# aminrezaee/mujoco_reinforcement_learning

Measured on NVIDIA B200. Metric: ppo_update_samples_per_sec, higher is better.
Workload: dtype bf16

## Files before the change

### mujoco_reinforcement_learning_b200/build.py

```python
from __future__ import annotations

import os
import subprocess
import sys
from concurrent.futures import ThreadPoolExecutor

HERE = os.path.dirname(os.path.abspath(__file__))
ROOT = os.path.dirname(HERE)
CSRC = os.path.join(HERE, "csrc")
INCLUDE = os.path.join(ROOT, "include")
BUILD_DIR = os.path.join(HERE, "build")
LIB_PATH = os.path.join(HERE, "libb200ppo.so")

NVCC_FLAGS = [
    "-gencode", "arch=compute_100a,code=sm_100a", "-lineinfo", "-O3", "-std=c++17",
    "-Xcompiler", "-fPIC", "-Xcompiler", "-fvisibility=hidden", f"-I{INCLUDE}", f"-I{CSRC}",
]


def _sources():
    return sorted(os.path.join(CSRC, f) for f in os.listdir(CSRC) if f.endswith(".cu"))


def _newest_input():
    deps = [os.path.join(CSRC, f) for f in os.listdir(CSRC)] + [os.path.join(INCLUDE, "b200ppo.h"), __file__]
    return max(os.path.getmtime(p) for p in deps)


def needs_build() -> bool:
    return not os.path.exists(LIB_PATH) or os.path.getmtime(LIB_PATH) < _newest_input()


def build_library(force: bool = False, verbose: bool = False) -> str:
    if not force and not needs_build():
        return LIB_PATH
    nvcc = os.environ.get("NVCC", "/usr/local/cuda/bin/nvcc")
    os.makedirs(BUILD_DIR, exist_ok=True)

    def compile_one(src):
        obj = os.path.join(BUILD_DIR, os.path.basename(src)[:-3] + ".o")
        cmd = [nvcc, *NVCC_FLAGS, "-c", src, "-o", obj]
        if verbose:
            cmd.insert(1, "-Xptxas=-v")
        res = subprocess.run(cmd, capture_output=True, text=True)
        if res.returncode != 0:
            raise RuntimeError(f"nvcc failed for {src}:\n{res.stdout}\n{res.stderr}")
        if verbose:
            sys.stderr.write(res.stderr)
        return obj

    with ThreadPoolExecutor(max_workers=min(8, os.cpu_count() or 1)) as ex:
        objs = list(ex.map(compile_one, _sources()))
    tmp = LIB_PATH + ".tmp"
    res = subprocess.run([nvcc, "-shared", "-gencode", "arch=compute_100a,code=sm_100a", "-o", tmp, *objs, "-ldl"],
                         capture_output=True, text=True)
    if res.returncode != 0:
        raise RuntimeError(f"link failed:\n{res.stdout}\n{res.stderr}")
    os.replace(tmp, LIB_PATH)
    return LIB_PATH


if __name__ == "__main__":
    path = build_library(force="--force" in sys.argv, verbose="-v" in sys.argv)
    print(path)
```

### mujoco_reinforcement_learning_b200/csrc/adam.cu

```cuda
#include <math.h>

#include "adam.cuh"

namespace b200ppo {

__device__ __forceinline__ void adam_update(float& p, float g, float& m, float& v, const AdamScalars& s) {
  m = __fadd_rn(m, __fmul_rn(s.one_minus_b1, __fsub_rn(g, m)));
  v = __fadd_rn(__fmul_rn(v, s.b2), __fmul_rn(__fmul_rn(s.one_minus_b2, g), g));
  const float denom = __fadd_rn(__fdiv_rn(__fsqrt_rn(v), s.bc2_sqrt), s.eps);
  p = __fadd_rn(p, __fmul_rn(s.neg_step_size, __fdiv_rn(m, denom)));
}

__global__ void __launch_bounds__(256)
adam_kernel(float* __restrict__ params, const float* __restrict__ grads, int n_partials, int64_t partial_stride,
            float* __restrict__ exp_avg, float* __restrict__ exp_avg_sq, int64_t n, int64_t seg_split,
            AdamScalars s0, AdamScalars s1, float* __restrict__ grad_out) {
  const int64_t tid = int64_t(blockIdx.x) * blockDim.x + threadIdx.x;
  const int64_t nthreads = int64_t(gridDim.x) * blockDim.x;
  const int64_t n4 = n >> 2;
  for (int64_t i = tid; i < n4; i += nthreads) {
    float4 g = *reinterpret_cast<const float4*>(grads + 4 * i);
    for (int k = 1; k < n_partials; ++k) {
      const float4 h = *reinterpret_cast<const float4*>(grads + k * partial_stride + 4 * i);
      g.x += h.x; g.y += h.y; g.z += h.z; g.w += h.w;
    }
    float4 p = *reinterpret_cast<float4*>(params + 4 * i);
    float4 m = *reinterpret_cast<float4*>(exp_avg + 4 * i);
    float4 v = *reinterpret_cast<float4*>(exp_avg_sq + 4 * i);
    const int64_t e = 4 * i;
    adam_update(p.x, g.x, m.x, v.x, e + 0 < seg_split ? s0 : s1);
    adam_update(p.y, g.y, m.y, v.y, e + 1 < seg_split ? s0 : s1);
    adam_update(p.z, g.z, m.z, v.z, e + 2 < seg_split ? s0 : s1);
    adam_update(p.w, g.w, m.w, v.w, e + 3 < seg_split ? s0 : s1);
    *reinterpret_cast<float4*>(params + 4 * i) = p;
    *reinterpret_cast<float4*>(exp_avg + 4 * i) = m;
    *reinterpret_cast<float4*>(exp_avg_sq + 4 * i) = v;
    if (grad_out != nullptr) *reinterpret_cast<float4*>(grad_out + 4 * i) = g;
  }
  for (int64_t e = 4 * n4 + tid; e < n; e += nthreads) {
    float g = grads[e];
    for (int k = 1; k < n_partials; ++k) g += grads[k * partial_stride + e];
    float p = params[e], m = exp_avg[e], v = exp_avg_sq[e];
    adam_update(p, g, m, v, e < seg_split ? s0 : s1);
    params[e] = p; exp_avg[e] = m; exp_avg_sq[e] = v;
    if (grad_out != nullptr) grad_out[e] = g;
  }
}

__device__ __forceinline__ void add_partials(float4& g, const float* __restrict__ grads, int k0, int n_partials, int64_t partial_stride, int64_t i) {
  constexpr int NB = 8;
  for (; k0 < n_partials; k0 += NB) {
    float4 h[NB];
#pragma unroll
    for (int j = 0; j < NB; ++j)
      if (k0 + j < n_partials) h[j] = __ldg(reinterpret_cast<const float4*>(grads + int64_t(k0 + j) * partial_stride + 4 * i));
#pragma unroll
    for (int j = 0; j < NB; ++j)
      if (k0 + j < n_partials) { g.x += h[j].x; g.y += h[j].y; g.z += h[j].z; g.w += h[j].w; }
  }
}

struct CastTable {
  int64_t begin[2 * B200PPO_MAX_LAYERS], end[2 * B200PPO_MAX_LAYERS];
  __nv_bfloat16* dst[2 * B200PPO_MAX_LAYERS];
  int in[2 * B200PPO_MAX_LAYERS], pitch[2 * B200PPO_MAX_LAYERS];
  int count;
};

__device__ __forceinline__ void combine_losses(const LossCombine& lc, float* s_lc, float* s_scr) {
  const int tid = threadIdx.x;
  const float s = combine_partials<256>(lc.partials, unsigned(lc.n_cta), 2 + lc.act_dim, tid, s_scr);
  if (tid < 2 + lc.act_dim) s_lc[tid] = tid < 2 ? s : s - lc.ent_coef * lc.rank_share / float(lc.act_dim);
  if (tid == 0 && lc.losses_out != nullptr) {
    float ent = 0.f;
    for (int j = 0; j < lc.act_dim; ++j) ent += 0.5f + 0.91893853320467274178f + logf(expf(lc.logstd[j]));
    ent /= float(lc.act_dim);
    lc.losses_out[0] = -s * lc.inv_global_batch - lc.ent_coef * ent * lc.rank_share;
  }
  if (tid == 1 && lc.losses_out != nullptr) lc.losses_out[1] = s * lc.inv_global_batch;
  __syncthreads();
}

__device__ __forceinline__ bool peer_exchange_barrier(const PeerSrc& ps) {
  const int q = threadIdx.x;
  int timed_out = 0;
  if (q < ps.world && q != ps.rank) {
    if (blockIdx.x == 0) {
      if (ps.local_out != nullptr) {
        const long long t0 = clock64();
        unsigned d;
        do {
          asm volatile("ld.acquire.gpu.global.u32 %0, [%1];" : "=r"(d) : "l"(ps.done_counter) : "memory");
        } while (int(d - ps.done_target) < 0 && clock64() - t0 <= ps.timeout_cycles);
      }
      __threadfence_system();
      asm volatile("st.release.sys.global.u32 [%0], %1;" ::"l"(ps.flags_peer[q] + ps.rank), "r"(ps.seq) : "memory");
    }
    const long long t0 = clock64();
    unsigned v;
    do {
      asm volatile("ld.acquire.sys.global.u32 %0, [%1];" : "=r"(v) : "l"(ps.flags_local + q) : "memory");
      if (clock64() - t0 > ps.timeout_cycles) {
        if (ps.err != nullptr) atomicMax(ps.err, B200PPO_ERRFLAG_PEER_TIMEOUT);
        timed_out = 1;
        break;
      }
    } while (int(v - ps.seq) < 0);
  }
  return __syncthreads_or(timed_out) == 0;
}

__device__ __forceinline__ float4 ld_peer4(const float* p) {
  float4 r;
  asm volatile("ld.volatile.global.v4.f32 {%0,%1,%2,%3}, [%4];" : "=f"(r.x), "=f"(r.y), "=f"(r.z), "=f"(r.w) : "l"(p) : "memory");
  return r;
}

template <bool PEERS>
__global__ void __launch_bounds__(256, 3)
adam_cast_kernel(float* __restrict__ params, const float* __restrict__ grads, int n_partials, int64_t partial_stride,
                 float* __restrict__ exp_avg, float* __restrict__ exp_avg_sq, int64_t n, int64_t seg_split, AdamScalars s0,
                 AdamScalars s1, const __grid_constant__ CastTable ct, const __grid_constant__ LossCombine lc,
                 const __grid_constant__ PeerSrc ps) {
  __shared__ float s_lc[64];
  __shared__ float s_scr[256];
  pdl_wait_then_release();
  const int64_t tid = int64_t(blockIdx.x) * blockDim.x + threadIdx.x;
  const int64_t nthreads = int64_t(gridDim.x) * blockDim.x;
  const int64_t n4 = n >> 2;
  const bool lc_owner = lc.partials != nullptr && int64_t(blockIdx.x) == ((lc.logstd_off >> 2) / blockDim.x) % gridDim.x;
  if (lc_owner) combine_losses(lc, s_lc, s_scr);
  float4 g_local = make_float4(0.f, 0.f, 0.f, 0.f);
  bool fused = false;
  if constexpr (PEERS) {
    fused = ps.local_out != nullptr;
    if (fused) {
      if (tid < n4) {
        g_local = __ldg(reinterpret_cast<const float4*>(grads + 4 * tid));
        add_partials(g_local, grads, 1, n_partials, partial_stride, tid);
        if (lc_owner && 4 * tid + 3 >= lc.logstd_off && 4 * tid < lc.logstd_off + lc.act_dim) {
          const int64_t r = 4 * tid - lc.logstd_off;
          if (r + 0 >= 0 && r + 0 < lc.act_dim) g_local.x = s_lc[2 + r + 0];
          if (r + 1 >= 0 && r + 1 < lc.act_dim) g_local.y = s_lc[2 + r + 1];
          if (r + 2 >= 0 && r + 2 < lc.act_dim) g_local.z = s_lc[2 + r + 2];
          if (r + 3 >= 0 && r + 3 < lc.act_dim) g_local.w = s_lc[2 + r + 3];
        }
        *reinterpret_cast<float4*>(ps.local_out + 4 * tid) = g_local;
      }
      __threadfence();
      __syncthreads();
      if (threadIdx.x == 0) atomicAdd(ps.done_counter, 1u);
    }
    if (!peer_exchange_barrier(ps)) return;
    if (blockIdx.x == 0 && threadIdx.x < 2 && ps.losses_out != nullptr) {
      float l = 0.f;
      for (int r = 0; r < ps.world; ++r) {
        float t;
        asm volatile("ld.volatile.global.f32 %0, [%1];" : "=f"(t) : "l"(ps.src[r] + n + threadIdx.x) : "memory");
        l += t;
      }
      ps.losses_out[threadIdx.x] = l;
    }
  }
  for (int64_t i = tid; i < n4; i += nthreads) {
    const float4 p0 = *reinterpret_cast<float4*>(params + 4 * i);
    const float4 m0 = *reinterpret_cast<float4*>(exp_avg + 4 * i);
    const float4 v0 = *reinterpret_cast<float4*>(exp_avg_sq + 4 * i);
    float4 g;
    if constexpr (PEERS) {
      float4 h[kMaxPeers];
#pragma unroll
      for (int r = 0; r < kMaxPeers; ++r)
        if (r < ps.world) h[r] = (fused && r == ps.rank) ? g_local : ld_peer4(ps.src[r] + 4 * i);
      g = h[0];
#pragma unroll
      for (int r = 1; r < kMaxPeers; ++r)
        if (r < ps.world) { g.x += h[r].x; g.y += h[r].y; g.z += h[r].z; g.w += h[r].w; }
    } else {
      g = *reinterpret_cast<const float4*>(grads + 4 * i);
    }
    if constexpr (!PEERS) add_partials(g, grads, 1, n_partials, partial_stride, i);
    if (!PEERS && lc_owner && 4 * i + 3 >= lc.logstd_off && 4 * i < lc.logstd_off + lc.act_dim) {
      const int64_t r = 4 * i - lc.logstd_off;
      if (r + 0 >= 0 && r + 0 < lc.act_dim) g.x = s_lc[2 + r + 0];
      if (r + 1 >= 0 && r + 1 < lc.act_dim) g.y = s_lc[2 + r + 1];
      if (r + 2 >= 0 && r + 2 < lc.act_dim) g.z = s_lc[2 + r + 2];
      if (r + 3 >= 0 && r + 3 < lc.act_dim) g.w = s_lc[2 + r + 3];
    }
    float4 p = p0, m = m0, v = v0;
    const int64_t e = 4 * i;
    adam_update(p.x, g.x, m.x, v.x, e + 0 < seg_split ? s0 : s1);
    adam_update(p.y, g.y, m.y, v.y, e + 1 < seg_split ? s0 : s1);
    adam_update(p.z, g.z, m.z, v.z, e + 2 < seg_split ? s0 : s1);
    adam_update(p.w, g.w, m.w, v.w, e + 3 < seg_split ? s0 : s1);
    *reinterpret_cast<float4*>(params + 4 * i) = p;
    *reinterpret_cast<float4*>(exp_avg + 4 * i) = m;
    *reinterpret_cast<float4*>(exp_avg_sq + 4 * i) = v;
    int k = -1;
#pragma unroll 1
    for (int c = 0; c < ct.count; ++c)
      if (e >= ct.begin[c] && e < ct.end[c]) k = c;
    if (k >= 0 && (ct.in[k] & 3) == 0 && (ct.pitch[k] & 3) == 0 && e + 3 < ct.end[k]) {
      const uint32_t in = uint32_t(ct.in[k]), rel = uint32_t(e - ct.begin[k]);
      const uint32_t o = rel / in, c2 = rel - o * in;
      const __nv_bfloat162 lo = __floats2bfloat162_rn(p.x, p.y), hi = __floats2bfloat162_rn(p.z, p.w);
      uint2 w;
      w.x = *reinterpret_cast<const uint32_t*>(&lo);
      w.y = *reinterpret_cast<const uint32_t*>(&hi);
      *reinterpret_cast<uint2*>(ct.dst[k] + int64_t(o) * ct.pitch[k] + c2) = w;
    } else if (k >= 0) {
      const float pv[4] = {p.x, p.y, p.z, p.w};
      const int in = ct.in[k];
      const int64_t rel = e - ct.begin[k];
#pragma unroll
      for (int j = 0; j < 4; ++j) {
        if (e + j >= ct.end[k]) break;
        const int o = int((rel + j) / in), c2 = int((rel + j) - int64_t(o) * in);
        ct.dst[k][int64_t(o) * ct.pitch[k] + c2] = __float2bfloat16_rn(pv[j]);
      }
    }
  }
}

__global__ void __launch_bounds__(256)
reduce_partials_kernel(const float* __restrict__ grads, int n_partials, int64_t partial_stride, int64_t n,
                       float* __restrict__ out, const __grid_constant__ LossCombine lc, int vec4) {
  __shared__ float s_lc[64];
  __shared__ float s_scr[256];
  pdl_wait_then_release();
  const int64_t tid = int64_t(blockIdx.x) * blockDim.x + threadIdx.x;
  const int64_t nthreads = int64_t(gridDim.x) * blockDim.x;
  const int64_t n4 = vec4 ? (n >> 2) : 0;
  const bool lc_owner = lc.partials != nullptr && int64_t(blockIdx.x) == (vec4 ? ((lc.logstd_off >> 2) / blockDim.x) % gridDim.x
                                                                               : (lc.logstd_off / blockDim.x) % gridDim.x);
  if (lc_owner) combine_losses(lc, s_lc, s_scr);
  for (int64_t i = tid; i < n4; i += nthreads) {
    float4 g = *reinterpret_cast<const float4*>(grads + 4 * i);
    add_partials(g, grads, 1, n_partials, partial_stride, i);
    if (lc_owner && 4 * i + 3 >= lc.logstd_off && 4 * i < lc.logstd_off + lc.act_dim) {
      const int64_t r = 4 * i - lc.logstd_off;
      if (r + 0 >= 0 && r + 0 < lc.act_dim) g.x = s_lc[2 + r + 0];
      if (r + 1 >= 0 && r + 1 < lc.act_dim) g.y = s_lc[2 + r + 1];
      if (r + 2 >= 0 && r + 2 < lc.act_dim) g.z = s_lc[2 + r + 2];
      if (r + 3 >= 0 && r + 3 < lc.act_dim) g.w = s_lc[2 + r + 3];
    }
    *reinterpret_cast<float4*>(out + 4 * i) = g;
  }
  for (int64_t e = 4 * n4 + tid; e < n; e += nthreads) {
    float g = grads[e];
    for (int k = 1; k < n_partials; ++k) g += grads[k * partial_stride + e];
    if (lc_owner && e >= lc.logstd_off && e < lc.logstd_off + lc.act_dim) g = s_lc[2 + (e - lc.logstd_off)];
    out[e] = g;
  }
}

AdamScalars make_adam_scalars(double lr, double beta1, double beta2, double eps, int64_t step) {
  AdamScalars s;
  const double bc1 = 1.0 - pow(beta1, double(step));
  const double bc2 = 1.0 - pow(beta2, double(step));
  s.one_minus_b1 = float(1.0 - beta1);
  s.b2 = float(beta2);
  s.one_minus_b2 = float(1.0 - beta2);
  s.bc2_sqrt = float(sqrt(bc2));
  s.eps = float(eps);
  s.neg_step_size = float(-(lr / bc1));
  return s;
}

static inline unsigned ew_grid(int64_t work_items) {
  int64_t blocks = (work_items + 255) / 256;
  const int64_t cap = int64_t(num_sms()) * 8;
  if (blocks > cap) blocks = cap;
  return unsigned(blocks < 1 ? 1 : blocks);
}

int launch_adam(float* params, const float* grads, int n_partials, int64_t partial_stride, float* exp_avg,
                float* exp_avg_sq, int64_t n, int64_t seg_split, const AdamScalars& s0, const AdamScalars& s1,
                float* grad_out, cudaStream_t st) {
  if (n == 0) return B200PPO_OK;
  adam_kernel<<<ew_grid((n + 3) / 4), 256, 0, st>>>(params, grads, n_partials, partial_stride, exp_avg, exp_avg_sq, n,
                                                    seg_split, s0, s1, grad_out);
  B2_LAUNCH_CHECK();
  return B200PPO_OK;
}

int adam_cast_grid(int64_t n) { return int(ew_grid(n / 4)); }

int launch_adam_cast(float* params, const float* grads, int n_partials, int64_t partial_stride, float* exp_avg,
                     float* exp_avg_sq, int64_t n, int64_t seg_split, const AdamScalars& s0, const AdamScalars& s1,
                     const WeightCastGroup& casts, const LossCombine& lc, cudaStream_t st, const PeerSrc* peers) {
  if (n == 0) return B200PPO_OK;
  const PeerSrc no_peers{};
  B2_CHECK_ARG(lc.partials == nullptr || (lc.act_dim + 2 <= 64 && lc.logstd_off % 4 == 0), "loss combine: act_dim <= 62");
  B2_CHECK_ARG(n % 4 == 0, "fused Adam + cast expects the padded flat parameter buffer");
  CastTable ct{};
  ct.count = casts.count;
  for (int k = 0; k < casts.count; ++k) {
    const WeightCast& w = casts.w[k];
    ct.begin[k] = w.src - params;
    ct.end[k] = ct.begin[k] + int64_t(w.out) * w.in;
    B2_CHECK_ARG(ct.begin[k] >= 0 && ct.end[k] <= n, "weight cast source outside the parameter buffer");
    ct.dst[k] = w.dst;
    ct.in[k] = w.in; ct.pitch[k] = w.pitch;
  }
  B2_CHECK_ARG(peers == nullptr || peers->local_out == nullptr || int64_t(ew_grid(n / 4)) * 256 >= n / 4,
               "fused reduce + exchange: one element per thread");
  if (peers != nullptr && peers->world > 0)
    B2_CUDA(launch_pdl(adam_cast_kernel<true>, dim3(ew_grid(n / 4)), dim3(256), 0, st, params, grads, n_partials, partial_stride, exp_avg,
                       exp_avg_sq, n, seg_split, s0, s1, ct, lc, *peers));
  else
    B2_CUDA(launch_pdl(adam_cast_kernel<false>, dim3(ew_grid(n / 4)), dim3(256), 0, st, params, grads, n_partials, partial_stride, exp_avg,
                       exp_avg_sq, n, seg_split, s0, s1, ct, lc, no_peers));
  B2_LAUNCH_CHECK();
  return B200PPO_OK;
}

int launch_reduce_partials(const float* grads, int n_partials, int64_t partial_stride, int64_t n, float* out,
                           cudaStream_t st, const LossCombine* lc) {
  if (n == 0) return B200PPO_OK;
  const LossCombine none{};
  const int vec4 = (n % 4 == 0 && partial_stride % 4 == 0 && aligned16(grads) && aligned16(out) && (lc == nullptr || lc->logstd_off % 4 == 0)) ? 1 : 0;
  B2_CUDA(launch_pdl(reduce_partials_kernel, dim3(ew_grid(vec4 ? n / 4 : n)), dim3(256), 0, st, grads, n_partials, partial_stride, n, out,
                     lc ? *lc : none, vec4));
  B2_LAUNCH_CHECK();
  return B200PPO_OK;
}

__global__ void __launch_bounds__(256)
polyak_kernel(float* __restrict__ target, const float* __restrict__ source, int64_t n, float one_minus_tau, float tau) {
  const int64_t tid = int64_t(blockIdx.x) * blockDim.x + threadIdx.x;
  const int64_t nthreads = int64_t(gridDim.x) * blockDim.x;
  const int64_t n4 = ((reinterpret_cast<uintptr_t>(target) | reinterpret_cast<uintptr_t>(source)) & 15u) == 0 ? (n >> 2) : 0;
  for (int64_t i = tid; i < n4; i += nthreads) {
    float4 t = ldg_stream4(target + 4 * i);
    const float4 s = ldg_stream4(source + 4 * i);
    t.x = __fadd_rn(__fmul_rn(t.x, one_minus_tau), __fmul_rn(s.x, tau));
    t.y = __fadd_rn(__fmul_rn(t.y, one_minus_tau), __fmul_rn(s.y, tau));
    t.z = __fadd_rn(__fmul_rn(t.z, one_minus_tau), __fmul_rn(s.z, tau));
    t.w = __fadd_rn(__fmul_rn(t.w, one_minus_tau), __fmul_rn(s.w, tau));
    stg_stream4(target + 4 * i, t);
  }
  for (int64_t e = 4 * n4 + tid; e < n; e += nthreads)
    target[e] = __fadd_rn(__fmul_rn(target[e], one_minus_tau), __fmul_rn(source[e], tau));
}

}

using namespace b200ppo;

extern "C" B2_EXPORT int b200ppo_polyak_update(float* target, const float* source, int64_t n, double tau, b200ppo_stream stream) {
  B2_CHECK_ARG(target && source && n >= 0, "b200ppo_polyak_update: bad argument");
  if (n == 0) return B200PPO_OK;
  polyak_kernel<<<ew_grid((n + 3) / 4), 256, 0, static_cast<cudaStream_t>(stream)>>>(target, source, n, float(1.0 - tau), float(tau));
  B2_LAUNCH_CHECK();
  return B200PPO_OK;
}

extern "C" B2_EXPORT int b200ppo_adam_step(float* params, const float* grads, int32_t n_partials, int64_t partial_stride,
                                 float* exp_avg, float* exp_avg_sq, int64_t n, double lr, double beta1, double beta2,
                                 double eps, int64_t step, b200ppo_stream stream) {
  B2_CHECK_ARG(params && grads && exp_avg && exp_avg_sq, "b200ppo_adam_step: null pointer");
  B2_CHECK_ARG(n >= 0 && n_partials >= 1 && step >= 1, "b200ppo_adam_step: bad n/n_partials/step");
  B2_CHECK_ARG(aligned16(params) && aligned16(grads) && aligned16(exp_avg) && aligned16(exp_avg_sq) &&
                   (n_partials == 1 || partial_stride % 4 == 0),
               "b200ppo_adam_step: buffers must be 16-byte aligned");
  const AdamScalars s = make_adam_scalars(lr, beta1, beta2, eps, step);
  return launch_adam(params, grads, n_partials, partial_stride, exp_avg, exp_avg_sq, n, n, s, s, nullptr,
                     static_cast<cudaStream_t>(stream));
}
```

### mujoco_reinforcement_learning_b200/csrc/common.cuh

```cuda
#pragma once
#include <cuda_runtime.h>
#include <stdint.h>
#include <stdio.h>
#include <stdlib.h>

#include <utility>

#include "b200ppo.h"

#define B2_EXPORT __attribute__((visibility("default")))

namespace b200ppo {

void set_error(const char* fmt, ...);
void count_launch();

#define B2_CHECK_ARG(cond, ...)           \
  do {                                    \
    if (!(cond)) {                        \
      ::b200ppo::set_error(__VA_ARGS__);  \
      return B200PPO_EINVAL;              \
    }                                     \
  } while (0)

#define B2_CUDA(expr)                                                                              \
  do {                                                                                             \
    cudaError_t _e = (expr);                                                                       \
    if (_e != cudaSuccess) {                                                                       \
      ::b200ppo::set_error("%s:%d: %s failed: %s", __FILE__, __LINE__, #expr, cudaGetErrorString(_e)); \
      return B200PPO_ECUDA;                                                                        \
    }                                                                                              \
  } while (0)

#define B2_LAUNCH_CHECK()                \
  do {                                   \
    ::b200ppo::count_launch();           \
    B2_CUDA(cudaGetLastError());         \
  } while (0)

#define B2_TRY(expr)            \
  do {                          \
    int _r = (expr);            \
    if (_r != B200PPO_OK) return _r; \
  } while (0)

inline int num_sms() {
  static int sms = 0;
  if (sms == 0) {
    int dev = 0;
    if (cudaGetDevice(&dev) != cudaSuccess || cudaDeviceGetAttribute(&sms, cudaDevAttrMultiProcessorCount, dev) != cudaSuccess)
      sms = 148;
  }
  return sms;
}

inline bool pdl_enabled() {
  static const bool on = []() {
    const char* e = getenv("B200PPO_PDL");
    return !(e != nullptr && e[0] == '0');
  }();
  return on;
}

template <typename... KArgs, typename... Args>
inline cudaError_t launch_pdl(void (*kernel)(KArgs...), dim3 grid, dim3 block, size_t smem, cudaStream_t st, Args&&... args) {
  cudaLaunchConfig_t cfg{};
  cfg.gridDim = grid;
  cfg.blockDim = block;
  cfg.dynamicSmemBytes = smem;
  cfg.stream = st;
  cudaLaunchAttribute at[1];
  at[0].id = cudaLaunchAttributeProgrammaticStreamSerialization;
  at[0].val.programmaticStreamSerializationAllowed = 1;
  cfg.attrs = at;
  cfg.numAttrs = pdl_enabled() ? 1 : 0;
  return cudaLaunchKernelEx(&cfg, kernel, std::forward<Args>(args)...);
}

__device__ __forceinline__ void pdl_wait_then_release() {
  asm volatile("griddepcontrol.wait;" ::: "memory");
  asm volatile("griddepcontrol.launch_dependents;" ::: "memory");
}

inline bool aligned16(const void* p) { return (reinterpret_cast<uintptr_t>(p) & 15u) == 0; }

__device__ __forceinline__ float warp_sum(float v) {
#pragma unroll
  for (int o = 16; o > 0; o >>= 1) v += __shfl_xor_sync(0xffffffffu, v, o);
  return v;
}
__device__ __forceinline__ double warp_sum(double v) {
#pragma unroll
  for (int o = 16; o > 0; o >>= 1) v += __shfl_xor_sync(0xffffffffu, v, o);
  return v;
}

__device__ __forceinline__ float4 ldg_stream4(const float* p) {
  float4 r;
  asm volatile("ld.global.nc.L1::no_allocate.v4.f32 {%0,%1,%2,%3}, [%4];" : "=f"(r.x), "=f"(r.y), "=f"(r.z), "=f"(r.w) : "l"(p));
  return r;
}
__device__ __forceinline__ void stg_stream4(float* p, float4 v) {
  asm volatile("st.global.L1::no_allocate.v4.f32 [%0], {%1,%2,%3,%4};" ::"l"(p), "f"(v.x), "f"(v.y), "f"(v.z), "f"(v.w) : "memory");
}


template <int THREADS>
__device__ __forceinline__ float combine_partials(const float* partials, unsigned n_cta, int width, int c_out, float* s_scratch) {
  constexpr int COLS = 64;
  constexpr int PARTS = THREADS / COLS;
  const int tid = threadIdx.x, c = tid % COLS, part = tid / COLS;
  float s = 0.f;
  if (c < width && part < PARTS) {
    const unsigned per = (n_cta + PARTS - 1) / PARTS;
    const unsigned k0 = part * per, k1 = min(n_cta, k0 + per);
    unsigned k = k0;
    for (; k + 16 <= k1; k += 16) {
      float v[16];
#pragma unroll
      for (int j = 0; j < 16; ++j) v[j] = __ldcg(partials + size_t(k + j) * width + c);
#pragma unroll
      for (int j = 0; j < 16; ++j) s += v[j];
    }
    for (; k < k1; ++k) s += __ldcg(partials + size_t(k) * width + c);
  }
  s_scratch[tid] = s;
  __syncthreads();
  float total = 0.f;
  if (tid < width) {
    for (int p = 0; p < PARTS; ++p) total += s_scratch[p * COLS + tid];
  }
  (void)c_out;
  return total;
}

}
```

### mujoco_reinforcement_learning_b200/csrc/tc_wgrad.cu

```cuda
#include <algorithm>

#include "tc_common.cuh"

namespace b200ppo {

constexpr int kWg2MaxTiles = 24;
constexpr int WG2_STAGES = 6;
constexpr int WG2_STAGE_BYTES = TC_A_BYTES + 128 * TC_BK * 2;
constexpr int WG2_ONES_BYTES = 4096;

struct Wg2Tile {
  int prob, m0, n0, nw, bias;
  int pair_begin, splits, k_tiles_per_split;
};

struct Wg2Group {
  TcProblem p[kMaxTcProblems];
  Wg2Tile tile[kWg2MaxTiles];
  int count, n_tiles, max_splits;
};

__global__ void __cluster_dims__(2, 1, 1) __launch_bounds__(TC_THREADS, 1) tc_wgrad2_kernel(const __grid_constant__ Wg2Group grp) {
  constexpr uint32_t TMEM_COLS = 512;
  constexpr uint32_t BIAS_COL = 256;
  extern __shared__ uint8_t smem_raw[];
  uint8_t* smem = smem_raw + ((1024u - (smem_u32(smem_raw) & 1023u)) & 1023u);
  uint8_t* ring = smem;
  uint8_t* ones = smem + WG2_STAGES * WG2_STAGE_BYTES;
  uint64_t* full_bar = reinterpret_cast<uint64_t*>(ones + WG2_ONES_BYTES);
  uint64_t* empty_bar = full_bar + WG2_STAGES;
  uint64_t* done_bar = empty_bar + WG2_STAGES;
  uint32_t* tmem_slot = reinterpret_cast<uint32_t*>(done_bar + 1);

  const int warp = threadIdx.x >> 5, lane = threadIdx.x & 31;
  const uint32_t rank = cluster_ctarank();
  const int pair = int(blockIdx.x) >> 1;
  int ti = 0;
#pragma unroll 1
  for (int i = 1; i < grp.n_tiles; ++i)
    if (pair >= grp.tile[i].pair_begin) ti = i;
  const Wg2Tile T = grp.tile[ti];
  const int split = pair - T.pair_begin;
  const TcProblem& P = grp.p[T.prob];
  const int total_kt = (P.K + TC_BK - 1) / TC_BK;
  const int kt_begin = split * T.k_tiles_per_split;
  const int kt_end = min(total_kt, kt_begin + T.k_tiles_per_split);
  const bool has_k = kt_end > kt_begin;
  const int nw_half = T.nw >> 1;
  const uint32_t stage_tx = 2u * uint32_t(TC_A_BYTES + nw_half * TC_BK * 2);

  for (int i = threadIdx.x; i < WG2_ONES_BYTES / 4; i += TC_THREADS) reinterpret_cast<uint32_t*>(ones)[i] = 0x3F803F80u;
  fence_proxy_async_smem();
  if (warp == 1 && lane == 0) {
    for (int s = 0; s < WG2_STAGES; ++s) { mbar_init(&full_bar[s], 1); mbar_init(&empty_bar[s], 1); }
    mbar_init(done_bar, 1);
    mbar_init_fence();
  } else if (warp == 2) {
    tmem_alloc<2, TMEM_COLS>(tmem_slot);
  }
  tc_fence_before();
  __syncthreads();
  cluster_sync_all();
  tc_fence_after();
  const uint32_t tmem_base = *tmem_slot;
  pdl_wait_then_release();

  if (warp == 0) {
    if (lane == 0 && has_k) {
      const int ma = T.m0 + int(rank) * TC_BM;
      const int nb = T.n0 + int(rank) * nw_half;
      for (int kt = kt_begin, it = 0; kt < kt_end; ++kt, ++it) {
        const int s = it % WG2_STAGES;
        const uint32_t ph = (it / WG2_STAGES) & 1;
        mbar_wait(&empty_bar[s], ph ^ 1);
        if (rank == 0) mbar_expect_tx(&full_bar[s], stage_tx);
        const uint32_t leader_full = mapa_u32(smem_u32(&full_bar[s]), 0);
        uint8_t* a = ring + s * WG2_STAGE_BYTES;
        uint8_t* b = a + TC_A_BYTES;
        tma_load_2d_pair(a, &P.tmA, leader_full, ma, kt * TC_BK);
        tma_load_2d_pair(a + 64 * TC_BK * 2, &P.tmA, leader_full, ma + 64, kt * TC_BK);
        tma_load_2d_pair(b, &P.tmB, leader_full, nb, kt * TC_BK);
        if (nw_half > 64) tma_load_2d_pair(b + 64 * TC_BK * 2, &P.tmB, leader_full, nb + 64, kt * TC_BK);
      }
    }
  } else if (warp == 1) {
    if (lane == 0 && rank == 0 && has_k) {
      const uint32_t idesc = umma_idesc(2 * TC_BM, T.nw, true, true);
      constexpr uint32_t idesc_bias = umma_idesc(2 * TC_BM, 32, true, false);
      const uint32_t lbo = TC_BK * 128;
      const uint32_t ones_addr = smem_u32(ones);
      for (int kt = kt_begin, it = 0; kt < kt_end; ++kt, ++it) {
        const int s = it % WG2_STAGES;
        const uint32_t ph = (it / WG2_STAGES) & 1;
        mbar_wait(&full_bar[s], ph);
        tc_fence_after();
        const uint32_t a_addr = smem_u32(ring + s * WG2_STAGE_BYTES), b_addr = a_addr + TC_A_BYTES;
#pragma unroll
        for (int k = 0; k < TC_BK / 16; ++k) {
          const uint64_t ad = umma_desc(a_addr + k * 2048, lbo, 1024);
          const uint32_t acc = (it > 0 || k > 0) ? 1u : 0u;
          umma2_bf16(tmem_base, ad, umma_desc(b_addr + k * 2048, lbo, 1024), idesc, acc);
          if (T.bias) umma2_bf16(tmem_base + BIAS_COL, ad, umma_desc(ones_addr + k * 32, 0, 1024), idesc_bias, acc);
        }
        umma2_commit(&empty_bar[s]);
      }
      umma2_commit(done_bar);
    }
  } else {
    const int q = warp & 3, half = (warp - 2) >> 2;
    const int m = T.m0 + int(rank) * TC_BM + q * 32 + lane;
    const bool row_ok = m < P.M;
    if (has_k) {
      mbar_wait(done_bar, 0);
      tc_fence_after();
    }
    float* outp = P.out_f32 + int64_t(split) * P.split_stride + int64_t(m) * P.ld_f32;
    const bool vec = (P.ld_f32 % 4 == 0) && (P.split_stride % 4 == 0) && ((reinterpret_cast<uintptr_t>(P.out_f32) & 15u) == 0);
    const int c_begin = half * nw_half, c_end = c_begin + nw_half;
    for (int c = c_begin; c < c_end; c += 16) {
      uint32_t v[16];
      if (has_k) {
        tmem_ld16(tmem_base + (uint32_t(q * 32) << 16) + uint32_t(c), v);
      } else {
#pragma unroll
        for (int j = 0; j < 16; ++j) v[j] = 0u;
      }
      const int n = T.n0 + c;
      if (!row_ok || n >= P.N) continue;
      if (vec && n + 16 <= P.N) {
#pragma unroll
        for (int u = 0; u < 4; ++u)
          reinterpret_cast<float4*>(outp + n)[u] = make_float4(__uint_as_float(v[4 * u]), __uint_as_float(v[4 * u + 1]),
                                                                __uint_as_float(v[4 * u + 2]), __uint_as_float(v[4 * u + 3]));
      } else {
#pragma unroll
        for (int j = 0; j < 16; ++j)
          if (n + j < P.N) outp[n + j] = __uint_as_float(v[j]);
      }
    }
    if (T.bias && half == 0 && P.bias_grad != nullptr) {
      uint32_t v[16];
      if (has_k) {
        tmem_ld16(tmem_base + (uint32_t(q * 32) << 16) + BIAS_COL, v);
      } else {
        v[0] = 0u;
      }
      if (row_ok) P.bias_grad[int64_t(split) * P.split_stride + m] = __uint_as_float(v[0]);
    }
    for (int z = split + T.splits; z < grp.max_splits; z += T.splits) {
      if (!row_ok) break;
      float* zp = P.out_f32 + int64_t(z) * P.split_stride + int64_t(m) * P.ld_f32;
      for (int c = c_begin; c < c_end; c += 4) {
        const int n = T.n0 + c;
        if (n >= P.N) break;
        if (vec && n + 4 <= P.N) *reinterpret_cast<float4*>(zp + n) = make_float4(0.f, 0.f, 0.f, 0.f);
        else
          for (int j = 0; j < 4; ++j)
            if (n + j < P.N) zp[n + j] = 0.f;
      }
      if (T.bias && half == 0 && P.bias_grad != nullptr) P.bias_grad[int64_t(z) * P.split_stride + m] = 0.f;
    }
    tc_fence_before();
  }
  __syncthreads();
  cluster_sync_all();
  if (warp == 2) {
    tc_fence_after();
    tmem_dealloc<2, TMEM_COLS>(tmem_base);
  }
}

int launch_tc_wgrad2(const TcGroup& g, int max_split, cudaStream_t st, int* split_out) {
  Wg2Group w{};
  w.count = g.count;
  int64_t K = 0;
  for (int i = 0; i < g.count; ++i) {
    const TcProblem& p = g.p[i];
    B2_CHECK_ARG(p.a_mn_major && p.b_mn_major && p.out_f32 != nullptr, "pair weight-gradient kernel: MN-major operands, fp32 output");
    B2_CHECK_ARG(i == 0 || p.K == K, "pair weight-gradient kernel: all problems share the batch dimension");
    K = p.K;
    w.p[i] = p;
    for (int m0 = 0; m0 < p.M; m0 += 2 * TC_BM)
      for (int n0 = 0; n0 < p.N; n0 += 256) {
        B2_CHECK_ARG(w.n_tiles < kWg2MaxTiles, "pair weight-gradient kernel: too many output blocks");
        const int rem = p.N - n0;
        w.tile[w.n_tiles++] = Wg2Tile{i, m0, n0, rem > 128 ? 256 : 128, n0 == 0 ? 1 : 0};
      }
  }
  if (w.n_tiles == 0) return B200PPO_OK;
  const int total_kt = int((K + TC_BK - 1) / TC_BK);
  const int pairs = num_sms() / 2;
  int max_sp = 1;
  for (int t = 0; t < w.n_tiles; ++t) w.tile[t].splits = std::max(1, std::min({pairs / w.n_tiles, max_split, total_kt}));
  int begin = 0;
  for (int t = 0; t < w.n_tiles; ++t) {
    Wg2Tile& T = w.tile[t];
    T.k_tiles_per_split = (total_kt + T.splits - 1) / T.splits;
    T.splits = (total_kt + T.k_tiles_per_split - 1) / T.k_tiles_per_split;
    T.pair_begin = begin;
    begin += T.splits;
    max_sp = std::max(max_sp, T.splits);
  }
  w.max_splits = max_sp;
  const int total_pairs = begin;
  constexpr int smem = 1024 + WG2_STAGES * WG2_STAGE_BYTES + WG2_ONES_BYTES + 256;
  static bool configured = false;
  if (!configured) {
    B2_CUDA(cudaFuncSetAttribute(tc_wgrad2_kernel, cudaFuncAttributeMaxDynamicSharedMemorySize, smem));
    configured = true;
  }
  B2_CUDA(launch_pdl(tc_wgrad2_kernel, dim3(2 * total_pairs), dim3(TC_THREADS), smem, st, w));
  B2_LAUNCH_CHECK();
  if (split_out) *split_out = max_sp;
  return B200PPO_OK;
}

}
```

Before: 263.2 million.

## Prefetch Adam state and combine losses before the PDL wait in optimizer kernel

Moves the loss-partial combine and the first loads of params and Adam moments, plus the cast-slot lookup, ahead of the programmatic-dependent-launch wait. This lets that work overlap the tail of the preceding weight-gradient kernel. The single-device path now uses 192-thread blocks, two elements per thread and a grid capped at twice the SM count. It also adds an optional globaltimer trace build and profiling script. Risks are higher register pressure from the held prefetch registers and fewer threads available for the combine step.

```diff
diff --git a/mujoco_reinforcement_learning_b200/build.py b/mujoco_reinforcement_learning_b200/build.py
--- a/mujoco_reinforcement_learning_b200/build.py
+++ b/mujoco_reinforcement_learning_b200/build.py
@@ -31,15 +31,16 @@
     return not os.path.exists(LIB_PATH) or os.path.getmtime(LIB_PATH) < _newest_input()
 
 
-def build_library(force: bool = False, verbose: bool = False) -> str:
-    if not force and not needs_build():
+def build_library(force: bool = False, verbose: bool = False, lib_path: str = LIB_PATH, extra_flags=()) -> str:
+    if not force and lib_path == LIB_PATH and not needs_build():
         return LIB_PATH
     nvcc = os.environ.get("NVCC", "/usr/local/cuda/bin/nvcc")
-    os.makedirs(BUILD_DIR, exist_ok=True)
+    build_dir = BUILD_DIR if lib_path == LIB_PATH else os.path.splitext(lib_path)[0] + "_obj"
+    os.makedirs(build_dir, exist_ok=True)
 
     def compile_one(src):
-        obj = os.path.join(BUILD_DIR, os.path.basename(src)[:-3] + ".o")
-        cmd = [nvcc, *NVCC_FLAGS, "-c", src, "-o", obj]
+        obj = os.path.join(build_dir, os.path.basename(src)[:-3] + ".o")
+        cmd = [nvcc, *NVCC_FLAGS, *extra_flags, "-c", src, "-o", obj]
         if verbose:
             cmd.insert(1, "-Xptxas=-v")
         res = subprocess.run(cmd, capture_output=True, text=True)
@@ -51,13 +52,13 @@
 
     with ThreadPoolExecutor(max_workers=min(8, os.cpu_count() or 1)) as ex:
         objs = list(ex.map(compile_one, _sources()))
-    tmp = LIB_PATH + ".tmp"
+    tmp = lib_path + ".tmp"
     res = subprocess.run([nvcc, "-shared", "-gencode", "arch=compute_100a,code=sm_100a", "-o", tmp, *objs, "-ldl"],
                          capture_output=True, text=True)
     if res.returncode != 0:
         raise RuntimeError(f"link failed:\n{res.stdout}\n{res.stderr}")
-    os.replace(tmp, LIB_PATH)
-    return LIB_PATH
+    os.replace(tmp, lib_path)
+    return lib_path
 
 
 if __name__ == "__main__":
diff --git a/mujoco_reinforcement_learning_b200/csrc/adam.cu b/mujoco_reinforcement_learning_b200/csrc/adam.cu
--- a/mujoco_reinforcement_learning_b200/csrc/adam.cu
+++ b/mujoco_reinforcement_learning_b200/csrc/adam.cu
@@ -1,6 +1,14 @@
 #include <math.h>
 
+#include <algorithm>
+
 #include "adam.cuh"
+
+#ifdef B200PPO_ADAM_TRACE
+#define ADAM_TRACE(...) __VA_ARGS__
+#else
+#define ADAM_TRACE(...)
+#endif
 
 namespace b200ppo {
 
@@ -65,20 +73,26 @@
   __nv_bfloat16* dst[2 * B200PPO_MAX_LAYERS];
   int in[2 * B200PPO_MAX_LAYERS], pitch[2 * B200PPO_MAX_LAYERS];
   int count;
+  ADAM_TRACE(unsigned long long* trace;)
 };
 
-__device__ __forceinline__ void combine_losses(const LossCombine& lc, float* s_lc, float* s_scr) {
+template <int THREADS>
+__device__ __forceinline__ float combine_losses(const LossCombine& lc, float* s_lc, float* s_logstd, float* s_scr) {
   const int tid = threadIdx.x;
-  const float s = combine_partials<256>(lc.partials, unsigned(lc.n_cta), 2 + lc.act_dim, tid, s_scr);
+  const float ls = tid < lc.act_dim ? lc.logstd[tid] : 0.f;
+  const float s = combine_partials<THREADS, 4>(lc.partials, unsigned(lc.n_cta), 2 + lc.act_dim, tid, s_scr);
   if (tid < 2 + lc.act_dim) s_lc[tid] = tid < 2 ? s : s - lc.ent_coef * lc.rank_share / float(lc.act_dim);
-  if (tid == 0 && lc.losses_out != nullptr) {
+  if (tid < lc.act_dim) s_logstd[tid] = ls;
+  __syncthreads();
+  float loss = 0.f;
+  if (tid == 0) {
     float ent = 0.f;
-    for (int j = 0; j < lc.act_dim; ++j) ent += 0.5f + 0.91893853320467274178f + logf(expf(lc.logstd[j]));
+    for (int j = 0; j < lc.act_dim; ++j) ent += 0.5f + 0.91893853320467274178f + logf(expf(s_logstd[j]));
     ent /= float(lc.act_dim);
-    lc.losses_out[0] = -s * lc.inv_global_batch - lc.ent_coef * ent * lc.rank_share;
-  }
-  if (tid == 1 && lc.losses_out != nullptr) lc.losses_out[1] = s * lc.inv_global_batch;
-  __syncthreads();
+    loss = -s * lc.inv_global_batch - lc.ent_coef * ent * lc.rank_share;
+  }
+  if (tid == 1) loss = s * lc.inv_global_batch;
+  return loss;
 }
 
 __device__ __forceinline__ bool peer_exchange_barrier(const PeerSrc& ps) {
@@ -116,20 +130,57 @@
   return r;
 }
 
+__host__ __device__ constexpr int adam_cast_threads(bool peers) { return peers ? 256 : 192; }
+
 template <bool PEERS>
-__global__ void __launch_bounds__(256, 3)
+__global__ void __launch_bounds__(adam_cast_threads(PEERS), PEERS ? 3 : 2)
 adam_cast_kernel(float* __restrict__ params, const float* __restrict__ grads, int n_partials, int64_t partial_stride,
                  float* __restrict__ exp_avg, float* __restrict__ exp_avg_sq, int64_t n, int64_t seg_split, AdamScalars s0,
                  AdamScalars s1, const __grid_constant__ CastTable ct, const __grid_constant__ LossCombine lc,
                  const __grid_constant__ PeerSrc ps) {
-  __shared__ float s_lc[64];
+  constexpr int EPT = PEERS ? 1 : 2;
+  constexpr int THREADS = adam_cast_threads(PEERS);
+  __shared__ float s_lc[64], s_logstd[64];
   __shared__ float s_scr[256];
-  pdl_wait_then_release();
+  ADAM_TRACE(const unsigned long long t_entry = globaltimer();)
   const int64_t tid = int64_t(blockIdx.x) * blockDim.x + threadIdx.x;
   const int64_t nthreads = int64_t(gridDim.x) * blockDim.x;
   const int64_t n4 = n >> 2;
+  auto cast_slot = [&](int64_t e) {
+    int k = -1;
+#pragma unroll 1
+    for (int c = 0; c < ct.count; ++c)
+      if (e >= ct.begin[c] && e < ct.end[c]) k = c;
+    return k;
+  };
+  float4 p0[EPT], m0[EPT], v0[EPT];
+  int k0[EPT];
+#pragma unroll
+  for (int j = 0; j < EPT; ++j) {
+    const int64_t i = tid + j * nthreads;
+    if (i < n4) {
+      p0[j] = *reinterpret_cast<const float4*>(params + 4 * i);
+      m0[j] = *reinterpret_cast<const float4*>(exp_avg + 4 * i);
+      v0[j] = *reinterpret_cast<const float4*>(exp_avg_sq + 4 * i);
+      k0[j] = cast_slot(4 * i);
+    }
+  }
   const bool lc_owner = lc.partials != nullptr && int64_t(blockIdx.x) == ((lc.logstd_off >> 2) / blockDim.x) % gridDim.x;
-  if (lc_owner) combine_losses(lc, s_lc, s_scr);
+  float loss = 0.f;
+  if (lc_owner) loss = combine_losses<THREADS>(lc, s_lc, s_logstd, s_scr);
+  ADAM_TRACE(__syncthreads(); const unsigned long long t_pro = globaltimer();)
+  pdl_wait_then_release();
+  ADAM_TRACE(const unsigned long long t_wait = globaltimer();)
+  if (lc_owner && threadIdx.x < 2 && lc.losses_out != nullptr) lc.losses_out[threadIdx.x] = loss;
+  auto take_logstd_grad = [&](float4& g, int64_t i) {
+    if (lc_owner && 4 * i + 3 >= lc.logstd_off && 4 * i < lc.logstd_off + lc.act_dim) {
+      const int64_t r = 4 * i - lc.logstd_off;
+      if (r + 0 >= 0 && r + 0 < lc.act_dim) g.x = s_lc[2 + r + 0];
+      if (r + 1 >= 0 && r + 1 < lc.act_dim) g.y = s_lc[2 + r + 1];
+      if (r + 2 >= 0 && r + 2 < lc.act_dim) g.z = s_lc[2 + r + 2];
+      if (r + 3 >= 0 && r + 3 < lc.act_dim) g.w = s_lc[2 + r + 3];
+    }
+  };
   float4 g_local = make_float4(0.f, 0.f, 0.f, 0.f);
   bool fused = false;
   if constexpr (PEERS) {
@@ -138,13 +189,7 @@
       if (tid < n4) {
         g_local = __ldg(reinterpret_cast<const float4*>(grads + 4 * tid));
         add_partials(g_local, grads, 1, n_partials, partial_stride, tid);
-        if (lc_owner && 4 * tid + 3 >= lc.logstd_off && 4 * tid < lc.logstd_off + lc.act_dim) {
-          const int64_t r = 4 * tid - lc.logstd_off;
-          if (r + 0 >= 0 && r + 0 < lc.act_dim) g_local.x = s_lc[2 + r + 0];
-          if (r + 1 >= 0 && r + 1 < lc.act_dim) g_local.y = s_lc[2 + r + 1];
-          if (r + 2 >= 0 && r + 2 < lc.act_dim) g_local.z = s_lc[2 + r + 2];
-          if (r + 3 >= 0 && r + 3 < lc.act_dim) g_local.w = s_lc[2 + r + 3];
-        }
+        take_logstd_grad(g_local, tid);
         *reinterpret_cast<float4*>(ps.local_out + 4 * tid) = g_local;
       }
       __threadfence();
@@ -162,10 +207,7 @@
       ps.losses_out[threadIdx.x] = l;
     }
   }
-  for (int64_t i = tid; i < n4; i += nthreads) {
-    const float4 p0 = *reinterpret_cast<float4*>(params + 4 * i);
-    const float4 m0 = *reinterpret_cast<float4*>(exp_avg + 4 * i);
-    const float4 v0 = *reinterpret_cast<float4*>(exp_avg_sq + 4 * i);
+  auto update = [&](int64_t i, float4 p, float4 m, float4 v, int k) {
     float4 g;
     if constexpr (PEERS) {
       float4 h[kMaxPeers];
@@ -178,16 +220,9 @@
         if (r < ps.world) { g.x += h[r].x; g.y += h[r].y; g.z += h[r].z; g.w += h[r].w; }
     } else {
       g = *reinterpret_cast<const float4*>(grads + 4 * i);
-    }
-    if constexpr (!PEERS) add_partials(g, grads, 1, n_partials, partial_stride, i);
-    if (!PEERS && lc_owner && 4 * i + 3 >= lc.logstd_off && 4 * i < lc.logstd_off + lc.act_dim) {
-      const int64_t r = 4 * i - lc.logstd_off;
-      if (r + 0 >= 0 && r + 0 < lc.act_dim) g.x = s_lc[2 + r + 0];
-      if (r + 1 >= 0 && r + 1 < lc.act_dim) g.y = s_lc[2 + r + 1];
-      if (r + 2 >= 0 && r + 2 < lc.act_dim) g.z = s_lc[2 + r + 2];
-      if (r + 3 >= 0 && r + 3 < lc.act_dim) g.w = s_lc[2 + r + 3];
-    }
-    float4 p = p0, m = m0, v = v0;
+      add_partials(g, grads, 1, n_partials, partial_stride, i);
+      take_logstd_grad(g, i);
+    }
     const int64_t e = 4 * i;
     adam_update(p.x, g.x, m.x, v.x, e + 0 < seg_split ? s0 : s1);
     adam_update(p.y, g.y, m.y, v.y, e + 1 < seg_split ? s0 : s1);
@@ -196,10 +231,6 @@
     *reinterpret_cast<float4*>(params + 4 * i) = p;
     *reinterpret_cast<float4*>(exp_avg + 4 * i) = m;
     *reinterpret_cast<float4*>(exp_avg_sq + 4 * i) = v;
-    int k = -1;
-#pragma unroll 1
-    for (int c = 0; c < ct.count; ++c)
-      if (e >= ct.begin[c] && e < ct.end[c]) k = c;
     if (k >= 0 && (ct.in[k] & 3) == 0 && (ct.pitch[k] & 3) == 0 && e + 3 < ct.end[k]) {
       const uint32_t in = uint32_t(ct.in[k]), rel = uint32_t(e - ct.begin[k]);
       const uint32_t o = rel / in, c2 = rel - o * in;
@@ -219,21 +250,38 @@
         ct.dst[k][int64_t(o) * ct.pitch[k] + c2] = __float2bfloat16_rn(pv[j]);
       }
     }
-  }
+  };
+#pragma unroll
+  for (int j = 0; j < EPT; ++j) {
+    const int64_t i = tid + j * nthreads;
+    if (i < n4) update(i, p0[j], m0[j], v0[j], k0[j]);
+  }
+  for (int64_t i = tid + EPT * nthreads; i < n4; i += nthreads)
+    update(i, *reinterpret_cast<const float4*>(params + 4 * i), *reinterpret_cast<const float4*>(exp_avg + 4 * i),
+           *reinterpret_cast<const float4*>(exp_avg_sq + 4 * i), cast_slot(4 * i));
+#ifdef B200PPO_ADAM_TRACE
+  __syncthreads();
+  if (threadIdx.x == 0 && blockIdx.x < kAdamTraceBlocks) {
+    unsigned long long* r = ct.trace + 1 + 4 * blockIdx.x;
+    r[0] = t_entry; r[1] = t_pro; r[2] = t_wait; r[3] = globaltimer();
+  }
+#endif
 }
 
 __global__ void __launch_bounds__(256)
 reduce_partials_kernel(const float* __restrict__ grads, int n_partials, int64_t partial_stride, int64_t n,
                        float* __restrict__ out, const __grid_constant__ LossCombine lc, int vec4) {
-  __shared__ float s_lc[64];
+  __shared__ float s_lc[64], s_logstd[64];
   __shared__ float s_scr[256];
-  pdl_wait_then_release();
   const int64_t tid = int64_t(blockIdx.x) * blockDim.x + threadIdx.x;
   const int64_t nthreads = int64_t(gridDim.x) * blockDim.x;
   const int64_t n4 = vec4 ? (n >> 2) : 0;
   const bool lc_owner = lc.partials != nullptr && int64_t(blockIdx.x) == (vec4 ? ((lc.logstd_off >> 2) / blockDim.x) % gridDim.x
                                                                                : (lc.logstd_off / blockDim.x) % gridDim.x);
-  if (lc_owner) combine_losses(lc, s_lc, s_scr);
+  float loss = 0.f;
+  if (lc_owner) loss = combine_losses<256>(lc, s_lc, s_logstd, s_scr);
+  pdl_wait_then_release();
+  if (lc_owner && threadIdx.x < 2 && lc.losses_out != nullptr) lc.losses_out[threadIdx.x] = loss;
   for (int64_t i = tid; i < n4; i += nthreads) {
     float4 g = *reinterpret_cast<const float4*>(grads + 4 * i);
     add_partials(g, grads, 1, n_partials, partial_stride, i);
@@ -253,6 +301,20 @@
     out[e] = g;
   }
 }
+
+#ifdef B200PPO_ADAM_TRACE
+static unsigned long long* g_adam_trace = nullptr;
+static int g_adam_trace_n = 0;
+static constexpr size_t kAdamTraceBytes = sizeof(unsigned long long) * kAdamTraceLaunches * kAdamTraceStride;
+
+unsigned long long* adam_trace_record() {
+  if (g_adam_trace == nullptr &&
+      (cudaMalloc(&g_adam_trace, kAdamTraceBytes) != cudaSuccess || cudaMemset(g_adam_trace, 0, kAdamTraceBytes) != cudaSuccess))
+    abort();
+  return g_adam_trace + int64_t(g_adam_trace_n % kAdamTraceLaunches) * kAdamTraceStride;
+}
+void adam_trace_advance() { ++g_adam_trace_n; }
+#endif
 
 AdamScalars make_adam_scalars(double lr, double beta1, double beta2, double eps, int64_t step) {
   AdamScalars s;
@@ -285,6 +347,12 @@
 }
 
 int adam_cast_grid(int64_t n) { return int(ew_grid(n / 4)); }
+
+static unsigned adam_cast_single_grid(int64_t n) {
+  constexpr int per_block = 2 * adam_cast_threads(false);
+  const int64_t blocks = (n / 4 + per_block - 1) / per_block;
+  return unsigned(std::max<int64_t>(1, std::min<int64_t>(blocks, 2 * num_sms())));
+}
 
 int launch_adam_cast(float* params, const float* grads, int n_partials, int64_t partial_stride, float* exp_avg,
                      float* exp_avg_sq, int64_t n, int64_t seg_split, const AdamScalars& s0, const AdamScalars& s1,
@@ -303,15 +371,17 @@
     ct.dst[k] = w.dst;
     ct.in[k] = w.in; ct.pitch[k] = w.pitch;
   }
+  ADAM_TRACE(ct.trace = adam_trace_record();)
   B2_CHECK_ARG(peers == nullptr || peers->local_out == nullptr || int64_t(ew_grid(n / 4)) * 256 >= n / 4,
                "fused reduce + exchange: one element per thread");
   if (peers != nullptr && peers->world > 0)
     B2_CUDA(launch_pdl(adam_cast_kernel<true>, dim3(ew_grid(n / 4)), dim3(256), 0, st, params, grads, n_partials, partial_stride, exp_avg,
                        exp_avg_sq, n, seg_split, s0, s1, ct, lc, *peers));
   else
-    B2_CUDA(launch_pdl(adam_cast_kernel<false>, dim3(ew_grid(n / 4)), dim3(256), 0, st, params, grads, n_partials, partial_stride, exp_avg,
+    B2_CUDA(launch_pdl(adam_cast_kernel<false>, dim3(adam_cast_single_grid(n)), dim3(adam_cast_threads(false)), 0, st, params, grads, n_partials, partial_stride, exp_avg,
                        exp_avg_sq, n, seg_split, s0, s1, ct, lc, no_peers));
   B2_LAUNCH_CHECK();
+  ADAM_TRACE(adam_trace_advance();)
   return B200PPO_OK;
 }
 
@@ -356,6 +426,22 @@
   return B200PPO_OK;
 }
 
+#ifdef B200PPO_ADAM_TRACE
+extern "C" B2_EXPORT int b200ppo_debug_adam_trace(unsigned long long* out, int32_t max_launches) {
+  adam_trace_record();
+  B2_CUDA(cudaDeviceSynchronize());
+  const int n = std::min({g_adam_trace_n, kAdamTraceLaunches, int(max_launches)});
+  for (int j = 0; j < n; ++j) {
+    const int rec = (g_adam_trace_n - n + j) % kAdamTraceLaunches;
+    B2_CUDA(cudaMemcpy(out + int64_t(j) * kAdamTraceStride, g_adam_trace + int64_t(rec) * kAdamTraceStride,
+                       sizeof(unsigned long long) * kAdamTraceStride, cudaMemcpyDeviceToHost));
+  }
+  B2_CUDA(cudaMemset(g_adam_trace, 0, kAdamTraceBytes));
+  g_adam_trace_n = 0;
+  return n;
+}
+#endif
+
 extern "C" B2_EXPORT int b200ppo_adam_step(float* params, const float* grads, int32_t n_partials, int64_t partial_stride,
                                  float* exp_avg, float* exp_avg_sq, int64_t n, double lr, double beta1, double beta2,
                                  double eps, int64_t step, b200ppo_stream stream) {
diff --git a/mujoco_reinforcement_learning_b200/csrc/common.cuh b/mujoco_reinforcement_learning_b200/csrc/common.cuh
--- a/mujoco_reinforcement_learning_b200/csrc/common.cuh
+++ b/mujoco_reinforcement_learning_b200/csrc/common.cuh
@@ -82,6 +82,17 @@
   asm volatile("griddepcontrol.launch_dependents;" ::: "memory");
 }
 
+#ifdef B200PPO_ADAM_TRACE
+constexpr int kAdamTraceLaunches = 64, kAdamTraceBlocks = 1024, kAdamTraceStride = 1 + 4 * kAdamTraceBlocks;
+unsigned long long* adam_trace_record();
+void adam_trace_advance();
+__device__ __forceinline__ unsigned long long globaltimer() {
+  unsigned long long t;
+  asm volatile("mov.u64 %0, %%globaltimer;" : "=l"(t));
+  return t;
+}
+#endif
+
 inline bool aligned16(const void* p) { return (reinterpret_cast<uintptr_t>(p) & 15u) == 0; }
 
 __device__ __forceinline__ float warp_sum(float v) {
@@ -105,26 +116,33 @@
 }
 
 
-template <int THREADS>
+template <int THREADS, int PARTS = THREADS / 64>
 __device__ __forceinline__ float combine_partials(const float* partials, unsigned n_cta, int width, int c_out, float* s_scratch) {
   constexpr int COLS = 64;
-  constexpr int PARTS = THREADS / COLS;
-  const int tid = threadIdx.x, c = tid % COLS, part = tid / COLS;
-  float s = 0.f;
-  if (c < width && part < PARTS) {
-    const unsigned per = (n_cta + PARTS - 1) / PARTS;
-    const unsigned k0 = part * per, k1 = min(n_cta, k0 + per);
-    unsigned k = k0;
-    for (; k + 16 <= k1; k += 16) {
-      float v[16];
+  static_assert(THREADS % COLS == 0 && PARTS >= 1, "whole slices of 64 threads");
+  const int tid = threadIdx.x, c = tid % COLS;
+  auto slice = [&](int part) {
+    float s = 0.f;
+    if (c < width) {
+      const unsigned per = (n_cta + PARTS - 1) / PARTS;
+      const unsigned k0 = part * per, k1 = min(n_cta, k0 + per);
+      unsigned k = k0;
+      for (; k + 16 <= k1; k += 16) {
+        float v[16];
 #pragma unroll
-      for (int j = 0; j < 16; ++j) v[j] = __ldcg(partials + size_t(k + j) * width + c);
+        for (int j = 0; j < 16; ++j) v[j] = __ldcg(partials + size_t(k + j) * width + c);
 #pragma unroll
-      for (int j = 0; j < 16; ++j) s += v[j];
+        for (int j = 0; j < 16; ++j) s += v[j];
+      }
+      for (; k < k1; ++k) s += __ldcg(partials + size_t(k) * width + c);
     }
-    for (; k < k1; ++k) s += __ldcg(partials + size_t(k) * width + c);
+    return s;
+  };
+  if constexpr (PARTS == THREADS / COLS) {
+    s_scratch[tid] = slice(tid / COLS);
+  } else {
+    for (int part = tid / COLS; part < PARTS; part += THREADS / COLS) s_scratch[part * COLS + c] = slice(part);
   }
-  s_scratch[tid] = s;
   __syncthreads();
   float total = 0.f;
   if (tid < width) {
diff --git a/mujoco_reinforcement_learning_b200/csrc/tc_wgrad.cu b/mujoco_reinforcement_learning_b200/csrc/tc_wgrad.cu
--- a/mujoco_reinforcement_learning_b200/csrc/tc_wgrad.cu
+++ b/mujoco_reinforcement_learning_b200/csrc/tc_wgrad.cu
@@ -18,6 +18,9 @@
   TcProblem p[kMaxTcProblems];
   Wg2Tile tile[kWg2MaxTiles];
   int count, n_tiles, max_splits;
+#ifdef B200PPO_ADAM_TRACE
+  unsigned long long* trace;
+#endif
 };
 
 __global__ void __cluster_dims__(2, 1, 1) __launch_bounds__(TC_THREADS, 1) tc_wgrad2_kernel(const __grid_constant__ Wg2Group grp) {
@@ -168,6 +171,9 @@
     tc_fence_after();
     tmem_dealloc<2, TMEM_COLS>(tmem_base);
   }
+#ifdef B200PPO_ADAM_TRACE
+  if (threadIdx.x == 0) atomicMax(grp.trace, globaltimer());
+#endif
 }
 
 int launch_tc_wgrad2(const TcGroup& g, int max_split, cudaStream_t st, int* split_out) {
@@ -203,6 +209,9 @@
   }
   w.max_splits = max_sp;
   const int total_pairs = begin;
+#ifdef B200PPO_ADAM_TRACE
+  w.trace = adam_trace_record();
+#endif
   constexpr int smem = 1024 + WG2_STAGES * WG2_STAGE_BYTES + WG2_ONES_BYTES + 256;
   static bool configured = false;
   if (!configured) {
diff --git a/profiles/adam_trace.py b/profiles/adam_trace.py
--- /dev/null
+++ b/profiles/adam_trace.py
@@ -0,0 +1,85 @@
+import argparse
+import ctypes as C
+import os
+import sys
+import tempfile
+
+import numpy as np
+import torch
+
+ROOT = os.path.dirname(os.path.dirname(os.path.abspath(__file__)))
+sys.path.insert(0, ROOT)
+from mujoco_reinforcement_learning_b200 import _lib, build as _build
+
+STRIDE = 1 + 4 * 1024
+MAX_LAUNCHES = 64
+
+
+def main():
+    ap = argparse.ArgumentParser()
+    ap.add_argument("--lib", help="a library built with -DB200PPO_ADAM_TRACE (default: build one into a temporary directory)")
+    ap.add_argument("--epochs", type=int, default=8)
+    ap.add_argument("--minibatches", type=int, default=5, help="minibatches per epoch (epochs x this <= 64)")
+    args = ap.parse_args()
+    assert args.epochs * args.minibatches <= MAX_LAUNCHES
+    lib_path = args.lib or _build.build_library(force=True, lib_path=os.path.join(tempfile.mkdtemp(), "libb200ppo.so"),
+                                                extra_flags=["-DB200PPO_ADAM_TRACE"])
+    _build.LIB_PATH = lib_path
+    lib = _lib.load()
+    read = lib.b200ppo_debug_adam_trace
+    read.restype, read.argtypes = C.c_int32, [C.c_void_p, C.c_int32]
+
+    import mujoco_reinforcement_learning_b200 as pkg
+    D, A, H, B = 376, 17, [256, 256], 32768
+    M = args.minibatches * B
+    run = pkg.Run(training_config=pkg.TrainingConfig(learning_rate=1e-4, batch_size=B, epochs_per_iteration=args.epochs),
+                  environment_config=pkg.EnvironmentConfig(maximum_timesteps=1, num_envs=M),
+                  network_config=pkg.NetworkConfig(input_shape=D, output_shape=A, linear_hidden_shapes=H, critic_hidden_shapes=H),
+                  device="cuda:0", gemm_precision="bf16")
+    torch.manual_seed(0)
+    eng = pkg.PPOAgent(run, max_batch=B).engine
+    g = torch.Generator(device="cuda").manual_seed(1)
+    obs = torch.randn(M, D, device="cuda", generator=g)
+    act = torch.randn(M, A, device="cuda", generator=g).clamp_(-3, 3)
+    logp, _, _ = eng.evaluate(obs[:B], act[:B])
+    logp = logp.repeat(args.minibatches)
+    adv, tgt = torch.randn(M, device="cuda", generator=g), torch.randn(M, device="cuda", generator=g)
+    hp = eng.hparams(1e-4, 1e-4, 0.1, 1e-4)
+    perms = lambda e: torch.stack([torch.randperm(M, device="cuda", generator=g) for _ in range(e)])
+
+    out = np.zeros((MAX_LAUNCHES, STRIDE), dtype=np.uint64)
+    eng.train(obs, act, logp, adv, tgt, perms(2), B, hp)
+    read(out.ctypes.data, MAX_LAUNCHES)
+    eng.train(obs, act, logp, adv, tgt, perms(args.epochs), B, hp)
+    n = read(out.ctypes.data, MAX_LAUNCHES)
+    print(f"{torch.cuda.get_device_name()}; {n} optimizer launches traced ({args.epochs} epochs x {args.minibatches} "
+          f"minibatches of {B} rows, Humanoid {D}-{H}-{A}, bf16)")
+
+    rows = []
+    for j in range(n):
+        rec = out[j].astype(np.int64)
+        blocks = rec[1:].reshape(-1, 4)
+        blocks = blocks[blocks[:, 0] != 0]
+        rows.append((blocks - rec[0]) / 1e3)
+    print(f"blocks per launch: {sorted(set(len(r) for r in rows))}; times in us relative to the last weight-gradient CTA's exit (W)")
+    names = ["entry", "prologue done", "wait returned", "exit"]
+    pooled = np.concatenate(rows)
+    q = lambda x: "  ".join(f"{v:7.2f}" for v in np.percentile(x, [0, 10, 50, 90, 100]))
+    print(f"{'':24s}  {'min':>7s}  {'p10':>7s}  {'p50':>7s}  {'p90':>7s}  {'max':>7s}   (all blocks of all launches)")
+    for c, name in enumerate(names):
+        print(f"  {name:22s}  {q(pooled[:, c])}")
+    print(f"  {'exit - wait returned':22s}  {q(pooled[:, 3] - pooled[:, 2])}")
+    print(f"  {'prologue done - entry':22s}  {q(pooled[:, 1] - pooled[:, 0])}")
+    print(f"share of blocks that entered before W: {np.mean(pooled[:, 0] < 0):.3f}")
+    last_exit = np.array([r[:, 3].max() for r in rows])
+    longest = np.array([(r[:, 3] - r[:, 2]).max() for r in rows])
+    first_wait = np.array([r[:, 2].min() for r in rows])
+    print(f"per launch, last block's exit - W (the optimizer's share of the critical path): {q(last_exit)}")
+    print(f"per launch, first wait return - W:                                            {q(first_wait)}")
+    print(f"per launch, longest block after its wait:                                     {q(longest)}")
+    slow = [int(np.argmax(r[:, 3] - r[:, 2])) for r in rows]
+    print(f"block with the longest post-wait time, per launch: {sorted(set(slow))}")
+
+
+if __name__ == "__main__":
+    main()
```

After: 266.4 million (median of 6 runs). +1.2%, better.
